# jtschwar/tomo_TV

Hardware: AMD Instinct MI355X
Metric: SART+TV Gvoxel-updates/s (ASD-POCS outer iterations x voxels, 512x512x512 x 90 tilts, at 1/2/4/8 GPU) (higher is better)
Workload: dtype f32; 1 GPU; ASD-POCS iteration (SART sweep beta0=0.25 + 10 TV-GD steps) on ONE 512x512x512 volume, 90 tilts -70..70 deg (headline SART+TV 512^3x90 = BASELINE configs[2] shape), 512 slices on rank 0; volume=512x512x512, slices_per_gpu=512, nray=512, nproj=90, sub_slab_engines_per_gpu=1, sart_chains_per_engine=1

## Files before the change

tomo_tv_amd/csrc/engine_options.inc:

```

int tomo_get_option(tomo_engine *e, const char *name, int *value)
{
    if (!e || !name || !value) return fail(TOMO_ERR_ARG, "null argument");
    if (std::strcmp(name, "fp_strip") == 0) { *value = e->fp_strip; return TOMO_OK; }
    if (std::strcmp(name, "fp_strip_ready") == 0) { *value = e->fs_ok ? 1 : 0; return TOMO_OK; }
    if (std::strcmp(name, "fp_strip_slots") == 0) { *value = e->fs_ok ? e->fs_kused : 0; return TOMO_OK; }
    if (std::strcmp(name, "fp_tile") == 0) { *value = e->fp_tile; return TOMO_OK; }
    if (std::strcmp(name, "bp_tile") == 0) { *value = e->bp_tile; return TOMO_OK; }
    if (std::strcmp(name, "bp_list") == 0) { *value = e->bp_list; return TOMO_OK; }
    if (std::strcmp(name, "fgp_pair") == 0) { *value = e->fgp_pair; return TOMO_OK; }
    if (std::strcmp(name, "fp_list") == 0) { *value = e->fp_list; return TOMO_OK; }
    if (std::strcmp(name, "fp_list_ready") == 0) { *value = e->fl_ok ? 1 : 0; return TOMO_OK; }
    if (std::strcmp(name, "bp_list_ready") == 0) { *value = e->bl_ok ? 1 : 0; return TOMO_OK; }
    if (std::strcmp(name, "fp_reuse") == 0) { *value = e->fp_reuse; return TOMO_OK; }
    if (std::strcmp(name, "art_chain_ready") == 0) { *value = e->art_chain_ok ? 1 : 0; return TOMO_OK; }
    if (std::strcmp(name, "sart_tile") == 0) { *value = e->sart_tile; return TOMO_OK; }
    if (std::strcmp(name, "sart_resident") == 0) { *value = e->sart_resident; return TOMO_OK; }
    if (std::strcmp(name, "sart_resident_ready") == 0) { *value = e->rs_ok ? 1 : 0; return TOMO_OK; }
    if (std::strcmp(name, "sart_resident_active") == 0) { *value = (e->rs_ok && e->sart_resident != 0) ? 1 : 0; return TOMO_OK; }
    if (std::strcmp(name, "sart_resident_spin") == 0) { *value = (int)std::min<uint32_t>(e->rs_spin_limit, 0x7FFFFFFFu); return TOMO_OK; }
    if (std::strcmp(name, "sart_resident_fallbacks") == 0) { *value = e->rs_fallbacks; return TOMO_OK; }
    if (std::strcmp(name, "sart_resident_fallback_chunks") == 0) { *value = e->rs_fallback_chunks; return TOMO_OK; }
    if (std::strcmp(name, "sart_resident_skip") == 0) { *value = e->rs_skip; return TOMO_OK; }
    if (std::strcmp(name, "sart_resident_last_code") == 0) { *value = e->rs_last_code; return TOMO_OK; }
    if (std::strcmp(name, "table_kib") == 0) { *value = (int)std::min<size_t>(e->table_bytes >> 10, 0x7FFFFFFF); return TOMO_OK; }
    if (std::strcmp(name, "create_ms") == 0) { *value = (int)std::min(e->create_ms + 0.5, 2147483647.0); return TOMO_OK; }
    if (std::strcmp(name, "tv_halo_fold") == 0) { *value = e->tv_halo_fold; return TOMO_OK; }
    if (std::strcmp(name, "form_fp") == 0) { *value = select_forms(e).fp; return TOMO_OK; }
    if (std::strcmp(name, "form_bp") == 0) { *value = select_forms(e).bp; return TOMO_OK; }
    if (std::strcmp(name, "form_sart") == 0) { *value = select_forms(e).sart; return TOMO_OK; }
    if (std::strcmp(name, "rccl_version") == 0) { *value = g_rccl.version; return TOMO_OK; }
    if (std::strcmp(name, "comm_rounds") == 0) { *value = (int)std::min<int64_t>(e->comm_rounds, 0x7FFFFFFF); return TOMO_OK; }
    return fail(TOMO_ERR_ARG, std::string("unknown option ") + name);
}

int tomo_set_option(tomo_engine *e, const char *name, int value)
{
    if (!e || !name) return fail(TOMO_ERR_ARG, "null argument");
    if (std::strcmp(name, "fgp_fused") == 0) { e->fgp_fused = value ? 1 : 0; return TOMO_OK; }
    if (std::strcmp(name, "fgp_pair") == 0) { e->fgp_pair = value ? 1 : 0; return TOMO_OK; }
    if (std::strcmp(name, "sart_fused") == 0) { e->sart_fused = value ? 1 : 0; return TOMO_OK; }
    if (std::strcmp(name, "fp_all_lpr") == 0) { e->fp_all_lpr = (value == 16 || value == 32) ? value : 0; return TOMO_OK; }
// ... 19 lines not shown
    if (std::strcmp(name, "fp_tile_chunks_per_pass") == 0) {
        if (value < 0 || e->ft_part || e->ft_part_aux || e->fs_part || e->fs_part_aux || e->fl_part || e->fl_part_aux) return fail(TOMO_ERR_STATE, "fp_tile_chunks_per_pass must be set before the first projection");
        e->ft_ncp_forced = value; e->ft_ncp = 0; e->fs_ncp = 0; e->fl_ncp = 0; return TOMO_OK;
    }
    if (std::strcmp(name, "fp_tile_scratch_mib") == 0) {
        if (value <= 0 || e->ft_part || e->ft_part_aux || e->fs_part || e->fs_part_aux || e->fl_part || e->fl_part_aux) return fail(TOMO_ERR_STATE, "fp_tile_scratch_mib must be positive and set before the first projection");
        e->ft_scratch_cap = (size_t)value << 20; e->ft_ncp = 0; e->fs_ncp = 0; e->fl_ncp = 0; return TOMO_OK;
    }
    if (std::strcmp(name, "tv_gnorm_slot") == 0) {
        if (value < 0 || value >= TOMO_S_COUNT) return fail(TOMO_ERR_ARG, "bad scalar slot");
        e->gnorm_slot = value; return TOMO_OK;
    }
    if (std::strcmp(name, "tv_tz") == 0) { e->tv_tz = value == 4 ? 4 : 8; return TOMO_OK; }
    if (std::strcmp(name, "tv_halo_fold") == 0) { e->tv_halo_fold = value < 0 ? -1 : (value ? 1 : 0); return TOMO_OK; }
    if (std::strcmp(name, "tv_march4") == 0) { e->tv_march4 = value ? 1 : 0; return TOMO_OK; }
    if (std::strcmp(name, "tv_yseg") == 0) { e->tv_yseg = value < 0 ? 0 : value; return TOMO_OK; }
    if (std::strcmp(name, "tv_recompute") == 0) { e->tv_recompute = value ? 1 : 0; return TOMO_OK; }
    if (std::strcmp(name, "tv_lds") == 0) { e->tv_lds = value; return TOMO_OK; }
    return fail(TOMO_ERR_ARG, std::string("unknown option ") + name);
}

int tomo_profile_enable(tomo_engine *e, int kernel, int on)
{
    NEED(e);
    if (kernel < 0 || kernel >= PROF_MAX_KERNELS) return fail(TOMO_ERR_ARG, "bad kernel id");
    HIPCHK(hipStreamSynchronize(e->stream));
    e->prof[kernel].on = on != 0;
    e->prof[kernel].stride = on > 1 ? (unsigned)on : 1u;
    e->prof[kernel].seen = 0;
    e->prof[kernel].used = 0;
// ... 74 lines not shown
```

tomo_tv_amd/csrc/engine_tv.inc:

```

static int field_ptr(tomo_engine *e, int field, float **out)
{
    if (field == TOMO_FIELD_FGP_D) return get_scratch(e, &e->tvg, out);
    if (field == TOMO_FIELD_FGP_P1) return get_scratch(e, &e->fgp_p[0], out);
    return get_vol_ro(e, field, out);
}

int tomo_bind_halo(tomo_engine *e, void *device_lo, void *device_hi)
{
    NEED(e);
    HIPCHK(hipStreamSynchronize(e->stream));
    e->halo_lo = device_lo ? (float *)device_lo : e->halo_lo_own;
    e->halo_hi = device_hi ? (float *)device_hi : e->halo_hi_own;
    return TOMO_OK;
}

int tomo_halo_pack(tomo_engine *e, int field, int last, void *device_dst)
{
    NEED(e);
    float *x; int rc; if ((rc = field_ptr(e, field, &x))) return rc;
    if (!device_dst) return fail(TOMO_ERR_ARG, "null destination");
    hipLaunchKernelGGL(k_halo_pack, dim3((unsigned)((e->npix + 255) / 256)), dim3(256), 0, e->stream, x, (float *)device_dst, (int)e->npix, e->sx, last ? e->nx - 1 : 0);
    LAUNCHCHK();
    return TOMO_OK;
// ... 93 lines not shown
        hipLaunchKernelGGL((k_tv_grad_lds<8, true, false>), grid, dim3(256), 0, e->stream, x, h, (float *)nullptr, (double *)nullptr, eps, e->n, e->nx, e->sx, yseg, e->d_part_tv);
    }
    LAUNCHCHK();
    return part_end(e, e->d_part_tv, TOMO_S_TV);
}

static int tv_rows_per_wave(const tomo_engine *e, int tz)
{
    if (e->tv_yseg > 0) return e->tv_yseg;
    const int64_t cols = (int64_t)((e->n + tz - 1) / tz) * (e->sxc / 64);
    int yseg = 32;
    while (yseg > TV_YSEG_MIN && cols * ((e->n + yseg - 1) / yseg) < TV_WAVES_WANTED) yseg >>= 1;
    return yseg;
}

static int tv_grad_impl(tomo_engine *e, float eps, bool with_tv, float *g_first = nullptr, float *g_last = nullptr)
{
    NEED(e);
    float *x, *g; int rc;
    if ((rc = get_vol(e, e->tv_target, &x))) return rc;
    if ((rc = get_scratch(e, &e->tvg, &g))) return rc;
    if ((rc = reduce_begin(e))) return rc;
    Halo h{e->halo_lo, e->halo_hi};
    if ((g_first || g_last) && !(e->tv_lds == 1 && e->tv_recompute)) return fail(TOMO_ERR_STATE, "gradient planes need the recompute form of the TV march (tv_lds = 1, tv_recompute = 1)");
    if (with_tv && e->tv_lds != 8 && e->tv_lds != 1) with_tv = false;
    if (with_tv) {
        if (!e->d_part_tv) { if ((rc = dev_alloc(e, ENGINE, (void **)&e->d_part_tv, NPART * sizeof(double), true))) return rc; }
        if ((rc = part_begin(e, e->d_part_tv))) return rc;
    }
    {
        ProfScope ps(e, TOMO_K_TV_GRAD);
        e->tv_last_eps = eps;
        double *part_tv = with_tv ? e->d_part_tv : nullptr;
        if (e->tv_lds == 1 && e->tv_recompute) {
            TvUpd gp{};
            gp.wrap_lo = g_last; gp.wrap_hi = g_first;
            const int tz = e->tv_tz == 4 ? 4 : 8, yseg = tv_rows_per_wave(e, tz);
            dim3 grid(tv_march_grid(e->n, tz, e->sxc / 64, (e->n + yseg - 1) / yseg));
            const bool edge = e->nx % 64 != 0 || e->n % 8 != 0;
            with_flag(with_tv, [&](auto W) {
                if (tz == 8 && e->tv_march4) with_flag(edge, [&](auto E) {
                    hipLaunchKernelGGL((k_tv_march4<8, W(), TVM_NORM, E()>), grid, dim3(256), 0, e->stream, x, h, e->d_part, eps, e->n, e->nx, e->sx, yseg, part_tv, gp);
                });
                else with_int<4, 8>(tz, [&](auto TZ) {
                    hipLaunchKernelGGL((k_tv_grad_reg<TZ(), W(), true, TVM_NORM>), grid, dim3(256), 0, e->stream, x, h, (float *)nullptr, e->d_part, eps, e->n, e->nx, e->sx, yseg, part_tv, gp);
                });
            });
        } else if (e->tv_lds == 1) {
            int yseg = 32;
            dim3 grid(tv_march_grid(e->n, 8, e->sxc / 64, (e->n + yseg - 1) / yseg));
            with_flag(with_tv, [&](auto W) {
                hipLaunchKernelGGL((k_tv_grad_reg<8, W()>), grid, dim3(256), 0, e->stream, x, h, g, e->d_part, eps, e->n, e->nx, e->sx, yseg, part_tv, TvUpd{});
            });
        } else if (e->tv_lds) {
            int yseg = 32;
            if (e->tv_lds == 16) {
                dim3 grid((unsigned)(((e->n + 15) / 16) * (e->sxc / 64)), (unsigned)((e->n + yseg - 1) / yseg));
                hipLaunchKernelGGL((k_tv_grad_lds<16, false>), grid, dim3(256), 0, e->stream, x, h, g, e->d_part, eps, e->n, e->nx, e->sx, yseg, (double *)nullptr);
            } else {
                dim3 grid((unsigned)(((e->n + 7) / 8) * (e->sxc / 64)), (unsigned)((e->n + yseg - 1) / yseg));
                with_flag(with_tv, [&](auto W) {
                    hipLaunchKernelGGL((k_tv_grad_lds<8, W()>), grid, dim3(256), 0, e->stream, x, h, g, e->d_part, eps, e->n, e->nx, e->sx, yseg, part_tv);
                });
            }
        } else {
            hipLaunchKernelGGL(k_tv_grad, dim3(tv_grid(e)), dim3(256), 0, e->stream, x, h, g, e->d_part, eps, e->n, e->nx, e->sx);
        }
    }
    LAUNCHCHK();
    if (with_tv && (rc = part_end(e, e->d_part_tv, TOMO_S_TV))) return rc;
    return reduce_end(e, TOMO_S_GNORM);
}

int tomo_tv_set_target(tomo_engine *e, int vol)
{
    NEED(e);
    float *x;
    int rc = get_vol(e, vol, &x);
    if (rc) return rc;
    e->tv_target = vol;
    return TOMO_OK;
}

int tomo_tv_grad(tomo_engine *e, float eps) { return tv_grad_impl(e, eps, false); }
int tomo_tv_grad_tv(tomo_engine *e, float eps)
{
// ... 21 lines not shown
}

static int halo_other_pair(tomo_engine *e, float **lo, float **hi)
{
    int rc;
    if (!e->halo_lo_alt) {
        if ((rc = dev_alloc(e, ENGINE, (void **)&e->halo_lo_alt, e->npix * sizeof(float), true))) return rc;
        if ((rc = dev_alloc(e, ENGINE, (void **)&e->halo_hi_alt, e->npix * sizeof(float), true))) return rc;
    }
    *lo = e->halo_lo == e->halo_lo_own ? e->halo_lo_alt : e->halo_lo_own;
    *hi = e->halo_hi == e->halo_hi_own ? e->halo_hi_alt : e->halo_hi_own;
    return TOMO_OK;
}

static int tv_update_impl(tomo_engine *e, float dPOCS, int clamp, int track_vol, int slot, bool wrap = false,
                          float *plane_last = nullptr, float *plane_first = nullptr, const float *hg_lo = nullptr, const float *hg_hi = nullptr)
{
    NEED(e);
    float *x, *g, *track = nullptr; int rc;
    if ((rc = get_vol(e, e->tv_target, &x))) return rc;
    if ((rc = get_scratch(e, &e->tvg, &g))) return rc;
    if (track_vol >= 0) {
        if (track_vol == e->tv_target) return fail(TOMO_ERR_ARG, "the tracked volume must differ from the one descended");
        if (slot < 0 || slot >= TOMO_S_COUNT) return fail(TOMO_ERR_ARG, "bad scalar slot");
        if ((rc = get_vol(e, track_vol, &track))) return rc;
        if ((rc = order_after_async(e))) return rc;
        if ((rc = reduce_begin(e))) return rc;
    }
    if (e->tv_lds == 1 && e->tv_recompute) {
        float *alt;
        if ((rc = get_scratch(e, &e->tv_alt, &alt))) return rc;
        const bool own_halo = e->halo_lo == e->halo_lo_own || e->halo_lo == e->halo_lo_alt;
        float *wl = plane_last, *wh = plane_first;
        if (wrap && own_halo && (rc = halo_other_pair(e, &wl, &wh))) return rc;
        Halo h{e->halo_lo, e->halo_hi};
        TvUpd up{alt, gnorm_ptr(e), dPOCS, clamp, track, wl, wh, slab_streams(e) ? 1 : 0, nullptr, nullptr, nullptr, nullptr};
        const bool fold = hg_lo && hg_hi && (e->tv_halo_fold < 0 ? e->sxc >= 128 : e->tv_halo_fold != 0) && own_halo && !wrap && e->tv_tz != 4 && e->tv_march4;
        if (fold) {
            up.hg_lo = hg_lo; up.hg_hi = hg_hi;
            if ((rc = halo_other_pair(e, &up.ho_lo, &up.ho_hi))) return rc;
        }
        {
            ProfScope ps(e, TOMO_K_TV_UPDATE);
            const int tz = e->tv_tz == 4 ? 4 : 8, yseg = tv_rows_per_wave(e, tz);
            dim3 grid(tv_march_grid(e->n, tz, e->sxc / 64, (e->n + yseg - 1) / yseg));
            const bool edge = e->nx % 64 != 0 || e->n % 8 != 0;
            if (tz == 8 && e->tv_march4) with_flag(edge, [&](auto E) { with_flag(track != nullptr, [&](auto T) { with_flag(up.stream != 0, [&](auto S) {
                hipLaunchKernelGGL((k_tv_march4<8, false, TVM_UPDATE, E(), T(), S()>), grid, dim3(256), 0, e->stream, x, h, e->d_part, e->tv_last_eps, e->n, e->nx, e->sx, yseg, (double *)nullptr, up);
            }); }); });
            else with_int<4, 8>(tz, [&](auto TZ) {
                hipLaunchKernelGGL((k_tv_grad_reg<TZ(), false, true, TVM_UPDATE>), grid, dim3(256), 0, e->stream, x, h, (float *)nullptr, e->d_part, e->tv_last_eps, e->n, e->nx, e->sx, yseg, (double *)nullptr, up);
            });
        }
        LAUNCHCHK();
        e->vol[e->tv_target] = alt; e->tv_alt = x;
        if (wrap && own_halo) { e->halo_lo = wl; e->halo_hi = wh; }
        else if (wrap) { if ((rc = tomo_halo_local(e, e->tv_target))) return rc; }
        if (fold) { e->halo_lo = up.ho_lo; e->halo_hi = up.ho_hi; }
        else if (hg_lo && hg_hi && (rc = tomo_tv_halo_apply(e, dPOCS, clamp, hg_lo, hg_hi))) return rc;
        return track ? reduce_end(e, slot) : TOMO_OK;
    }
    int64_t n4 = e->vol_elems() / 4;
// ... 76 lines not shown
    return TOMO_OK;
}

int tomo_tv(tomo_engine *e, int vol, float eps)
{
    int rc;
    if ((rc = tomo_halo_local(e, vol))) return rc;
    return tomo_tv_partial(e, vol, eps);
}

static int tv_gd_impl(tomo_engine *e, int ng, float dPOCS, float eps, int track_vol, int slot)
{
    int rc;
    if (!e) return fail(TOMO_ERR_ARG, "null engine");
    const bool fold_tv = ng > 0 && (e->tv_lds == 8 || e->tv_lds == 1);
    if (fold_tv) { if ((rc = tomo_halo_local(e, e->tv_target))) return rc; }
    else if ((rc = tomo_tv(e, e->tv_target, eps))) return rc;
    for (int g = 0; g < ng; ++g) {
        if ((rc = tv_grad_impl(e, eps, fold_tv && g == 0))) return rc;
        if ((rc = tv_update_impl(e, dPOCS, g == ng - 1, g == ng - 1 ? track_vol : -1, slot, g < ng - 1))) return rc;
    }
    if (ng <= 0) {
        if ((rc = tomo_positivity(e, e->tv_target))) return rc;
        if (track_vol >= 0) {
            if ((rc = tomo_diff_norm_sq(e, e->tv_target, track_vol, slot))) return rc;
            return tomo_copy_volume(e, track_vol, e->tv_target);
        }
    }
    return TOMO_OK;
}

int tomo_tv_gd(tomo_engine *e, int ng, float dPOCS, float eps) { return tv_gd_impl(e, ng, dPOCS, eps, -1, 0); }

int tomo_tv_gd_tracked(tomo_engine *e, int ng, float dPOCS, float eps, int track_vol, int slot)
{
// ... 155 lines not shown
```

tomo_tv_amd/csrc/kernels_common.hip.h:

```cpp
#pragma once

namespace tomo {


template <int V> struct VecOf;
template <> struct VecOf<1> { typedef float T; };
template <> struct VecOf<2> { typedef float T __attribute__((ext_vector_type(2))); };
template <> struct VecOf<4> { typedef float T __attribute__((ext_vector_type(4))); };

template <int V> __device__ __forceinline__ typename VecOf<V>::T vzero();
template <> __device__ __forceinline__ float vzero<1>() { return 0.f; }
template <> __device__ __forceinline__ VecOf<2>::T vzero<2>() { VecOf<2>::T v = {0.f, 0.f}; return v; }
template <> __device__ __forceinline__ VecOf<4>::T vzero<4>() { VecOf<4>::T v = {0.f, 0.f, 0.f, 0.f}; return v; }

template <int V> __device__ __forceinline__ float velem(const typename VecOf<V>::T &v, int i);
template <> __device__ __forceinline__ float velem<1>(const float &v, int) { return v; }
template <> __device__ __forceinline__ float velem<2>(const VecOf<2>::T &v, int i) { return v[i]; }
template <> __device__ __forceinline__ float velem<4>(const VecOf<4>::T &v, int i) { return v[i]; }

template <int V> __device__ __forceinline__ void vset(typename VecOf<V>::T &v, int i, float f);
template <> __device__ __forceinline__ void vset<1>(float &v, int, float f) { v = f; }
template <> __device__ __forceinline__ void vset<2>(VecOf<2>::T &v, int i, float f) { v[i] = f; }
template <> __device__ __forceinline__ void vset<4>(VecOf<4>::T &v, int i, float f) { v[i] = f; }

// ... 40 lines not shown
__global__ void k_finalize(double *__restrict__ part, double *__restrict__ dst)
{
    double v = part[threadIdx.x];
    part[threadIdx.x] = 0.0;
    __shared__ double red[NPART / 64];
    v = wave_sum(v);
    if ((threadIdx.x & 63) == 0) red[threadIdx.x >> 6] = v;
    __syncthreads();
    if (threadIdx.x == 0) {
        double s = 0;
        for (int i = 0; i < NPART / 64; ++i) s += red[i];
        *dst = s;
    }
}

__global__ __launch_bounds__(256) void k_transpose_in(const float *__restrict__ src, float *__restrict__ dst,
                                                       int ns, int64_t m, int sx)
{
    __shared__ float tile[32][33];
    int64_t m0 = (int64_t)blockIdx.x * 32;
    int s0 = blockIdx.y * 32;
    int tx = threadIdx.x & 31, ty = threadIdx.x >> 5;
    for (int r = ty; r < 32; r += 8) {
        int s = s0 + r;
        int64_t mm = m0 + tx;
        tile[r][tx] = (s < ns && mm < m) ? src[(int64_t)s * m + mm] : 0.f;
    }
    __syncthreads();
    for (int r = ty; r < 32; r += 8) {
        int64_t mm = m0 + r;
// ... 43 lines not shown
```

tomo_tv_amd/csrc/kernels_tv.hip.h:

```cpp
#pragma once

namespace tomo {

struct Halo { const float *lo; const float *hi; };

__device__ __forceinline__ float ldx(const float *__restrict__ x, const Halo &h, int pix, int s, int nx, int sx)
{
    if (s < 0) return h.lo[pix];
    if (s >= nx) return h.hi[pix];
    return x[(size_t)pix * sx + s];
}

__global__ void k_halo_pack(const float *__restrict__ x, float *__restrict__ dst, int npix, int sx, int s)
{
    int i = blockIdx.x * blockDim.x + threadIdx.x;
    if (i < npix) dst[i] = x[(size_t)i * sx + s];
}

__global__ void k_scalars_to_host(const double *__restrict__ src, double *__restrict__ host_dst, int n)
{
    int i = threadIdx.x;
    if (i < n) host_dst[i] = src[i];
}

// ... 172 lines not shown
}

__device__ __forceinline__ float tv_step_len(float dPOCS, const double *gnorm2) { return fminf(__fdiv_rn(dPOCS, (float)sqrt(*gnorm2)), 3.402823466e38f); }
__device__ __forceinline__ float tv_step(float c, float gv, float len) { return __fmaf_rn(-gv, len, c); }

constexpr int TVL_TZ = 8;
constexpr int TVL_PITCH = 66;

__device__ __forceinline__ float tv_ld(const float *__restrict__ x, const Halo &h, int pix, int s, int nx, int sx)
{
    const float *p = x + (size_t)pix * sx + s;
    p = (s < 0) ? h.lo + pix : p;
    p = (s >= nx) ? h.hi + pix : p;
    return *p;
}

template <int TZ, bool WITH_TV, bool GRAD = true>
__global__ __launch_bounds__(256) void k_tv_grad_lds(const float *__restrict__ x, Halo h, float *__restrict__ g,
                                                      double *__restrict__ part, float eps, int n, int nx, int sx,
                                                      int yseg, double *__restrict__ part_tv)
{
    __shared__ float ring[4][TZ + 2][TVL_PITCH];
    __shared__ float rinv[2][TZ + 1][TVL_PITCH];
    const int lane = threadIdx.x & 63, wave = threadIdx.x >> 6;
    const int nzb = (n + TZ - 1) / TZ;
    int bz = blockIdx.x % nzb;
    int bs = blockIdx.x / nzb;
    int y0 = blockIdx.y * yseg;
    int y1 = min(y0 + yseg, n);
    int z0 = bz * TZ, s0 = bs * 64;
// ... 75 lines not shown
        __syncthreads();
        block_accumulate(tvacc, part_tv);
    }
}

inline unsigned tv_march_grid(int n, int tz, int nchunk, int nys)
{
    const int nzb = (n + tz - 1) / tz;
    if ((nzb & 7) == 0) return 8u * (unsigned)(((int64_t)(nzb >> 3) * nchunk * nys + 3) / 4);
    return (unsigned)(((int64_t)nzb * nchunk * nys + 3) / 4);
}

enum { TVM_STORE = 0, TVM_NORM = 1, TVM_UPDATE = 2, TVM_VALUE = 3 };
struct TvUpd { float *x_out; const double *gnorm2; float dPOCS; int clamp; float *track; float *wrap_lo; float *wrap_hi;
               int stream;
               const float *hg_lo; const float *hg_hi; float *ho_lo; float *ho_hi; };

template <int TZ, bool WITH_TV, bool GRAD = true, int MODE = TVM_STORE>
__global__ __launch_bounds__(256) void k_tv_grad_reg(const float *__restrict__ x, Halo h, float *__restrict__ g,
                                                      double *__restrict__ part, float eps, int n, int nx, int sx,
                                                      int yseg, double *__restrict__ part_tv, TvUpd up = TvUpd{})
{
    const int lane = threadIdx.x & 63, wave = __builtin_amdgcn_readfirstlane(threadIdx.x >> 6);
    const int nzb = (n + TZ - 1) / TZ, nchunk = (nx + 63) >> 6   , nys = (n + yseg - 1) / yseg;
    double acc = 0.0, tvacc = 0.0;
    float nrm_ = 1.f;
    if (MODE == TVM_UPDATE) nrm_ = tv_step_len(up.dPOCS, up.gnorm2);
    int bs, bz, ys;
    bool live;
    if ((nzb & 7) == 0) {
        const int zpx = nzb >> 3;
// ... 134 lines not shown
        __syncthreads();
        block_accumulate(tvacc, part_tv);
    }
}

#ifndef TV4_PACKED
#define TV4_PACKED 1
#endif
#ifndef TV4_PACKED_EDGE
#define TV4_PACKED_EDGE 0
#endif
#ifndef TV4_UPD_WAVES
#define TV4_UPD_WAVES 4
#endif
#define TV4_OCC __attribute__((amdgpu_waves_per_eu((MODE == TVM_UPDATE && !TRACK) ? TV4_UPD_WAVES : 4, (MODE == TVM_UPDATE && !TRACK) ? TV4_UPD_WAVES : 8)))
template <int TZ, bool WITH_TV, int MODE, bool EDGE, bool TRACK = false, bool STREAM = false>
__global__ __launch_bounds__(256) TV4_OCC void k_tv_march4(const float *__restrict__ x, Halo h, double *__restrict__ part, float eps,
                                                    int n, int nx, int sx, int yseg, double *__restrict__ part_tv, TvUpd up)
{
    static_assert(MODE == TVM_NORM || MODE == TVM_UPDATE || MODE == TVM_VALUE, "modes without a stored gradient");
    static_assert(MODE != TVM_VALUE || WITH_TV, "the value mode sums the TV integrand");
    const int lane = threadIdx.x & 63, wave = __builtin_amdgcn_readfirstlane(threadIdx.x >> 6);
    const int nzb = (n + TZ - 1) / TZ, nchunk = (nx + 63) >> 6   , nys = (n + yseg - 1) / yseg;
    double acc = 0.0, tvacc = 0.0;
    float nrm_ = 1.f;
    if (MODE == TVM_UPDATE) nrm_ = tv_step_len(up.dPOCS, up.gnorm2);
    int bs, bz, ys;
    if ((nzb & 7) == 0) {
        const int zpx = nzb >> 3;
        const int64_t li = (int64_t)(blockIdx.x >> 3) * 4 + wave;
        bs = (int)(li % nchunk); bz = (int)(blockIdx.x & 7) * zpx + (int)((li / nchunk) % zpx); ys = (int)(li / ((int64_t)nchunk * zpx));
    } else {
        const int64_t item = (int64_t)blockIdx.x * 4 + wave;
        bs = (int)(item % nchunk); bz = (int)((item / nchunk) % nzb); ys = (int)(item / ((int64_t)nchunk * nzb));
    }
    if (ys < nys) {
        const int y0 = ys * yseg, y1 = min(y0 + yseg, n);
        const int z0 = bz * TZ, s0 = bs * 64, s = s0 + lane;
        int zc[TZ + 2];
#pragma unroll
        for (int j = 0; j < TZ + 2; ++j) { int z = (z0 - 1 + j) % n; zc[j] = z < 0 ? z + n : z; }
        int zl;
        { int z = (z0 - 1 + (lane < TZ + 2 ? lane : 0)) % n; zl = z < 0 ? z + n : z; }
        auto yrow = [&](int y) { int r = y % n; return r < 0 ? r + n : r; };
        float rows[4][TZ + 2], Ta[TZ + 1], Tb[TZ + 1];
        float pe[4], pf[4], pc[4];
        const bool lo_in = s0 > 0, hi_in = s0 + 64 < nx;
        const unsigned zls = (unsigned)zl * (unsigned)sx;
        const unsigned off_lo = lo_in ? zls + (unsigned)(s0 - 1) : (unsigned)zl, off_hi = hi_in ? zls + (unsigned)(s0 + 64) : (unsigned)zl;
        constexpr bool SOFF = !EDGE && !(WITH_TV && MODE == TVM_NORM);
        unsigned vb[TZ + 2];
#pragma unroll
        for (int j = 0; j < TZ + 2; ++j) vb[j] = ((unsigned)zc[j] * (unsigned)sx + (unsigned)s0 + (unsigned)lane) * 4u;
        unsigned eb_c = (zls + (unsigned)s0) * 4u, eb_lo = off_lo * 4u, eb_hi = off_hi * 4u;
        auto fetch = [&](int y, float *c, float &e_lo, float &e_hi, float &e_c) __attribute__((always_inline)) {
            int yy = yrow(y) * n;
            if (!EDGE) {
                const float *rowp = x + (size_t)yy * sx;
                if constexpr (SOFF) {
                    const SBase rb = sgpr_base(rowp);
#pragma unroll
                    for (int j = 0; j < TZ + 2; ++j) c[j] = ld_so(rb, vb[j]);
                    e_c = ld_so(rb, eb_c);
                    e_lo = ld_so(sgpr_base(lo_in ? rowp : h.lo + yy), eb_lo);
                    e_hi = ld_so(sgpr_base(hi_in ? rowp : h.hi + yy), eb_hi);
                } else {
#pragma unroll
                    for (int j = 0; j < TZ + 2; ++j) c[j] = (rowp + ((unsigned)zc[j] * (unsigned)sx + (unsigned)s0))[(unsigned)lane];
                    e_c = rowp[zls + (unsigned)s0];
                    e_lo = (lo_in ? rowp : h.lo + yy)[off_lo];
                    e_hi = (hi_in ? rowp : h.hi + yy)[off_hi];
                }
            } else {
#pragma unroll
                for (int j = 0; j < TZ + 2; ++j) c[j] = tv_ld(x, h, yy + zc[j], s, nx, sx);
                e_lo = tv_ld(x, h, yy + zl, s0 - 1, nx, sx);
                e_hi = tv_ld(x, h, yy + zl, s0 + 64, nx, sx);
                e_c = tv_ld(x, h, yy + zl, s0, nx, sx);
            }
        };
        const float vmin = up.clamp ? 0.f : -INFINITY;
        const bool planes = up.wrap_lo != nullptr && (EDGE || s0 == 0 || s0 + 64 == nx);
#define TV4_RINV(C, IP, JP, KP, RR, DD, D1, D2, D3)                                                       \
        {                                                                                                 \
            D1 = (C) - (IP); D2 = (C) - (JP); D3 = (C) - (KP);                                            \
            float q_ = __fmaf_rn(D3, D3, __fmaf_rn(D2, D2, __fmaf_rn(D1, D1, eps)));                      \
            RR = tv_rsqrt(q_);                                                                            \
// ... 132 lines not shown
                        else if (STREAM) __builtin_nontemporal_store(out[j], tr_e + (size_t)(j - 1) * sx + (unsigned)lane);
                        else (tr_e + (size_t)(j - 1) * sx)[(unsigned)lane] = out[j];
                    }
                }
            }
            if (planes) {
                if (s == 0) {
#pragma unroll
                    for (int j = 1; j <= TZ; ++j) if (!EDGE || z0 + j - 1 < n) up.wrap_hi[pix0 + (j - 1)] = out[j];
                }
                if (s == nx - 1) {
#pragma unroll
                    for (int j = 1; j <= TZ; ++j) if (!EDGE || z0 + j - 1 < n) up.wrap_lo[pix0 + (j - 1)] = out[j];
                }
            }
            if (MODE == TVM_UPDATE && up.hg_lo != nullptr && (EDGE || s0 == 0 || s0 + 64 == nx)) {
                if (!EDGE) {
                    const unsigned hp = (unsigned)(y * n) + (unsigned)zl;
                    if (lane >= 1 && lane <= TZ) {
                        if (s0 == 0) up.ho_lo[hp] = fmaxf(tv_step(pe0, up.hg_lo[hp], nrm_), vmin);
                        if (s0 + 64 == nx) up.ho_hi[hp] = fmaxf(tv_step(pf0, up.hg_hi[hp], nrm_), vmin);
                    }
                } else {
                    if (s == 0) {
#pragma unroll
                        for (int j = 1; j <= TZ; ++j)
                            if (z0 + j - 1 < n) up.ho_lo[pix0 + (j - 1)] = fmaxf(tv_step(h.lo[pix0 + (j - 1)], up.hg_lo[pix0 + (j - 1)], nrm_), vmin);
                    }
                    if (s == nx - 1) {
#pragma unroll
// ... 78 lines not shown
```

tomo_tv_amd/csrc/tomo_engine.hip:

```cpp
#include "../../include/tomo_hip.h"
#include "kernels.hip.h"
#include "sart_resident.hip.h"
#include "sysmat.h"
#include "resident.h"
#include "dev_pool.h"

#include <dlfcn.h>
#if __has_include(<rccl/rccl.h>)
#include <rccl/rccl.h>
#else
#define NCCL_UNIQUE_ID_BYTES 128
typedef struct ncclComm *ncclComm_t;
typedef struct { char internal[NCCL_UNIQUE_ID_BYTES]; } ncclUniqueId;
typedef enum { ncclSuccess = 0 } ncclResult_t;
typedef enum { ncclFloat32 = 7, ncclFloat64 = 8 } ncclDataType_t;
typedef enum { ncclSum = 0 } ncclRedOp_t;
#endif

#include <algorithm>
#include <atomic>
#include <chrono>
#include <cmath>
#include <condition_variable>
#include <functional>
// ... 89 lines not shown
    uint32_t *d_rptr = nullptr;
    uint2 *d_rent = nullptr;
    float *d_rowsum = nullptr, *d_rowinner = nullptr, *d_colsum_all = nullptr, *d_rowcross = nullptr;
    bool art_chain_ok = false;
    int art_chain = 1;
    CellD *d_cell = nullptr;
    uint32_t *d_wptr = nullptr;
    uint2 *d_went = nullptr;
    float lipschitz = 0.f, lipschitz_cimmino = 0.f;
    int sart_fused = 1;
    int tv_lds = 1, fp_all_lpr = 16;
    int tv_recompute = 1, tv_tz = 8;
    int tv_yseg = 0;
    int tv_march4 = 1;
    int tv_halo_fold = -1;
    int gnorm_slot = TOMO_S_GNORM;
    double *gnorm_override = nullptr;
    hipEvent_t ev_peer = nullptr;
    float tv_last_eps = 1e-6f;
    float *tv_alt = nullptr, *halo_lo_alt = nullptr, *halo_hi_alt = nullptr;
    SegItemD *d_seg_exec = nullptr;
    std::vector<uint32_t> h_seg_exec_ptr;
    uint32_t *d_row_first = nullptr, *d_row_nseg = nullptr;
    float *seg_partial = nullptr;
    uint32_t max_items = 0;
    bool seg_ready = false;
    std::vector<double> angles;
    float *sart_alt = nullptr;
    int fp_tile = 1, ft_tiles_z = 0, ft_ntiles = 0;
    uint32_t ft_nseg = 0;
// ... 86 lines not shown
    float *cg_coef = nullptr;
    float *tvg = nullptr;
    float *fgp_p[3] = {nullptr, nullptr, nullptr};
    float *fgp_q[3] = {nullptr, nullptr, nullptr};
    int fgp_fused = 1;
    int fgp_pair = 1;
    float *pdhg_p[3] = {nullptr, nullptr, nullptr}, *pdhg_alt[4] = {nullptr, nullptr, nullptr, nullptr}, *pdhg_q = nullptr;
    bool pdhg_begun = false;
    float *stage = nullptr;
    size_t stage_bytes = 0;
    double *d_scal = nullptr, *d_scal_own = nullptr, *d_part = nullptr, *d_part_aux = nullptr, *d_part_tv = nullptr;
    double *h_snap = nullptr;
    hipEvent_t ev_snap = nullptr;
    bool snap_pending = false;
    bool part_open[3] = {false, false, false};
    hipStream_t aux = nullptr;
    hipEvent_t ev_fork = nullptr, ev_join = nullptr;
    bool async_pending = false;
    struct CommRef *comm = nullptr;
    int64_t comm_rounds = 0;
    float *comm_send_first = nullptr, *comm_send_last = nullptr, *comm_g_lo = nullptr, *comm_g_hi = nullptr;
    float *comm_fgp = nullptr;
    double *comm_scal = nullptr;
    uint64_t vol_version[TOMO_VOL_SLOTS] = {};
    struct { int vol = -1; uint64_t ver = 0; } g_valid[2];
    int fp_reuse = 1;
    float *g_prev = nullptr;
    float *g_yk = nullptr;
    struct { bool valid = false; uint64_t ver = 0; } yk_claim;
    bool g_prev_valid = false, mom_p_ok = false;
// ... 134 lines not shown
}
static int part_begin(tomo_engine *e, double *part)
{
    bool &open = part_open(e, part);
    if (open) HIPCHK(hipMemsetAsync(part, 0, NPART * sizeof(double), e->stream));
    open = true;
    return TOMO_OK;
}
static int part_end(tomo_engine *e, double *part, int slot)
{
    hipLaunchKernelGGL(k_finalize, dim3(1), dim3(NPART), 0, e->stream, part, e->d_scal + slot);
    LAUNCHCHK();
    part_open(e, part) = false;
    return TOMO_OK;
}
static int reduce_begin(tomo_engine *e) { return part_begin(e, e->d_part); }
static int reduce_end(tomo_engine *e, int slot) { return part_end(e, e->d_part, slot); }

constexpr int TV_YSEG_MIN = 8, TV_WAVES_WANTED = 4096;
static int grid_1d(int64_t n4) { int64_t b = (n4 + 255) / 256; return (int)std::min<int64_t>(std::max<int64_t>(b, 1), 4096); }

#include "engine_launch.inc"
#include "engine_create.inc"

extern "C" {

#include "engine_api.inc"
#include "engine_tv.inc"
#include "engine_pdhg.inc"
#include "engine_comm.inc"
// ... 4 lines not shown
```

Measured before the change: 10.61 Gvoxel-updates/s.

## Fold TV gradient-norm finalize into update kernel and self-wrap first halo

In the plain single-GPU TV descent, the gradient-norm partial sums now go to double-buffered partial arrays. Each update kernel block reduces them itself, which removes the separate finalize launch and memset between norm and update passes. The next buffer is zeroed inside the norm kernel. The first norm pass can also read periodic x-neighbours directly from the volume and write the halo planes itself, skipping the separate halo_local step. The cost is a redundant per-block reduction of NPART doubles in every update block, plus extra template instantiations.

```diff
diff --git a/tomo_tv_amd/csrc/engine_options.inc b/tomo_tv_amd/csrc/engine_options.inc
--- a/tomo_tv_amd/csrc/engine_options.inc
+++ b/tomo_tv_amd/csrc/engine_options.inc
@@ -26,6 +26,19 @@
     if (std::strcmp(name, "table_kib") == 0) { *value = (int)std::min<size_t>(e->table_bytes >> 10, 0x7FFFFFFF); return TOMO_OK; }
     if (std::strcmp(name, "create_ms") == 0) { *value = (int)std::min(e->create_ms + 0.5, 2147483647.0); return TOMO_OK; }
     if (std::strcmp(name, "tv_halo_fold") == 0) { *value = e->tv_halo_fold; return TOMO_OK; }
+    if (std::strcmp(name, "tv_fold_sums") == 0) { *value = e->tv_fold_sums; return TOMO_OK; }
+    if (std::strcmp(name, "tv_self_wrap") == 0) { *value = e->tv_self_wrap; return TOMO_OK; }
+    if (std::strcmp(name, "tv_fold_sums_dirty") == 0) {
+        *value = -1;
+        if (!e->d_part_gn[0] || !e->d_part_gn[1]) return TOMO_OK;
+        double h[2 * NPART];
+        HIPCHK(hipSetDevice(e->device));
+        HIPCHK(hipStreamSynchronize(e->stream));
+        for (int k = 0; k < 2; ++k) HIPCHK(hipMemcpy(h + k * NPART, e->d_part_gn[k], NPART * sizeof(double), hipMemcpyDeviceToHost));
+        *value = 0;
+        for (double v : h) if (!(v == 0.0)) ++*value;
+        return TOMO_OK;
+    }
     if (std::strcmp(name, "form_fp") == 0) { *value = select_forms(e).fp; return TOMO_OK; }
     if (std::strcmp(name, "form_bp") == 0) { *value = select_forms(e).bp; return TOMO_OK; }
     if (std::strcmp(name, "form_sart") == 0) { *value = select_forms(e).sart; return TOMO_OK; }
@@ -75,6 +88,8 @@
     if (std::strcmp(name, "tv_tz") == 0) { e->tv_tz = value == 4 ? 4 : 8; return TOMO_OK; }
     if (std::strcmp(name, "tv_halo_fold") == 0) { e->tv_halo_fold = value < 0 ? -1 : (value ? 1 : 0); return TOMO_OK; }
     if (std::strcmp(name, "tv_march4") == 0) { e->tv_march4 = value ? 1 : 0; return TOMO_OK; }
+    if (std::strcmp(name, "tv_fold_sums") == 0) { e->tv_fold_sums = value < 0 ? -1 : (value ? 1 : 0); return TOMO_OK; }
+    if (std::strcmp(name, "tv_self_wrap") == 0) { e->tv_self_wrap = value < 0 ? -1 : (value ? 1 : 0); return TOMO_OK; }
     if (std::strcmp(name, "tv_yseg") == 0) { e->tv_yseg = value < 0 ? 0 : value; return TOMO_OK; }
     if (std::strcmp(name, "tv_recompute") == 0) { e->tv_recompute = value ? 1 : 0; return TOMO_OK; }
     if (std::strcmp(name, "tv_lds") == 0) { e->tv_lds = value; return TOMO_OK; }
diff --git a/tomo_tv_amd/csrc/engine_tv.inc b/tomo_tv_amd/csrc/engine_tv.inc
--- a/tomo_tv_amd/csrc/engine_tv.inc
+++ b/tomo_tv_amd/csrc/engine_tv.inc
@@ -131,13 +131,23 @@
     return yseg;
 }
 
-static int tv_grad_impl(tomo_engine *e, float eps, bool with_tv, float *g_first = nullptr, float *g_last = nullptr)
+static bool tv_plain_descent(const tomo_engine *e)
+{
+    const bool own_lo = e->halo_lo == e->halo_lo_own || (e->halo_lo_alt && e->halo_lo == e->halo_lo_alt);
+    const bool own_hi = e->halo_hi == e->halo_hi_own || (e->halo_hi_alt && e->halo_hi == e->halo_hi_alt);
+    return e->tv_lds == 1 && e->tv_recompute && e->tv_march4 && e->tv_tz != 4 && own_lo && own_hi &&
+           !e->gnorm_override && !e->comm && e->gnorm_slot == TOMO_S_GNORM;
+}
+
+static int tv_grad_impl(tomo_engine *e, float eps, bool with_tv, float *g_first = nullptr, float *g_last = nullptr,
+                        double *gn_part = nullptr, double *gn_zero = nullptr, bool self_wrap = false)
 {
     NEED(e);
     float *x, *g; int rc;
+    if ((gn_part || gn_zero || self_wrap) && (!tv_plain_descent(e) || g_first || g_last || (self_wrap && !with_tv))) return fail(TOMO_ERR_STATE, "not the whole-volume form of the TV descent");
     if ((rc = get_vol(e, e->tv_target, &x))) return rc;
     if ((rc = get_scratch(e, &e->tvg, &g))) return rc;
-    if ((rc = reduce_begin(e))) return rc;
+    if (!gn_part && (rc = reduce_begin(e))) return rc;
     Halo h{e->halo_lo, e->halo_hi};
     if ((g_first || g_last) && !(e->tv_lds == 1 && e->tv_recompute)) return fail(TOMO_ERR_STATE, "gradient planes need the recompute form of the TV march (tv_lds = 1, tv_recompute = 1)");
     if (with_tv && e->tv_lds != 8 && e->tv_lds != 1) with_tv = false;
@@ -152,12 +162,18 @@
         if (e->tv_lds == 1 && e->tv_recompute) {
             TvUpd gp{};
             gp.wrap_lo = g_last; gp.wrap_hi = g_first;
+            gp.zero_part = gn_zero;
+            if (self_wrap) { gp.ho_lo = e->halo_lo; gp.ho_hi = e->halo_hi; }
+            double *part = gn_part ? gn_part : e->d_part;
             const int tz = e->tv_tz == 4 ? 4 : 8, yseg = tv_rows_per_wave(e, tz);
             dim3 grid(tv_march_grid(e->n, tz, e->sxc / 64, (e->n + yseg - 1) / yseg));
             const bool edge = e->nx % 64 != 0 || e->n % 8 != 0;
-            with_flag(with_tv, [&](auto W) {
+            if (self_wrap) with_flag(edge, [&](auto E) {
+                hipLaunchKernelGGL((k_tv_march4<8, true, TVM_NORM, E(), false, false, true>), grid, dim3(256), 0, e->stream, x, h, part, eps, e->n, e->nx, e->sx, yseg, part_tv, gp);
+            });
+            else with_flag(with_tv, [&](auto W) {
                 if (tz == 8 && e->tv_march4) with_flag(edge, [&](auto E) {
-                    hipLaunchKernelGGL((k_tv_march4<8, W(), TVM_NORM, E()>), grid, dim3(256), 0, e->stream, x, h, e->d_part, eps, e->n, e->nx, e->sx, yseg, part_tv, gp);
+                    hipLaunchKernelGGL((k_tv_march4<8, W(), TVM_NORM, E()>), grid, dim3(256), 0, e->stream, x, h, part, eps, e->n, e->nx, e->sx, yseg, part_tv, gp);
                 });
                 else with_int<4, 8>(tz, [&](auto TZ) {
                     hipLaunchKernelGGL((k_tv_grad_reg<TZ(), W(), true, TVM_NORM>), grid, dim3(256), 0, e->stream, x, h, (float *)nullptr, e->d_part, eps, e->n, e->nx, e->sx, yseg, part_tv, gp);
@@ -186,7 +202,7 @@
     }
     LAUNCHCHK();
     if (with_tv && (rc = part_end(e, e->d_part_tv, TOMO_S_TV))) return rc;
-    return reduce_end(e, TOMO_S_GNORM);
+    return gn_part ? TOMO_OK : reduce_end(e, TOMO_S_GNORM);
 }
 
 int tomo_tv_set_target(tomo_engine *e, int vol)
@@ -238,10 +254,12 @@
 }
 
 static int tv_update_impl(tomo_engine *e, float dPOCS, int clamp, int track_vol, int slot, bool wrap = false,
-                          float *plane_last = nullptr, float *plane_first = nullptr, const float *hg_lo = nullptr, const float *hg_hi = nullptr)
+                          float *plane_last = nullptr, float *plane_first = nullptr, const float *hg_lo = nullptr, const float *hg_hi = nullptr,
+                          const double *gn_part = nullptr)
 {
     NEED(e);
     float *x, *g, *track = nullptr; int rc;
+    if (gn_part && (!tv_plain_descent(e) || track_vol >= 0 || hg_lo || hg_hi)) return fail(TOMO_ERR_STATE, "not the whole-volume form of the TV descent");
     if ((rc = get_vol(e, e->tv_target, &x))) return rc;
     if ((rc = get_scratch(e, &e->tvg, &g))) return rc;
     if (track_vol >= 0) {
@@ -259,6 +277,7 @@
         if (wrap && own_halo && (rc = halo_other_pair(e, &wl, &wh))) return rc;
         Halo h{e->halo_lo, e->halo_hi};
         TvUpd up{alt, gnorm_ptr(e), dPOCS, clamp, track, wl, wh, slab_streams(e) ? 1 : 0, nullptr, nullptr, nullptr, nullptr};
+        if (gn_part) { up.gnorm2 = gn_part; up.gnorm_out = e->d_scal + e->gnorm_slot; }
         const bool fold = hg_lo && hg_hi && (e->tv_halo_fold < 0 ? e->sxc >= 128 : e->tv_halo_fold != 0) && own_halo && !wrap && e->tv_tz != 4 && e->tv_march4;
         if (fold) {
             up.hg_lo = hg_lo; up.hg_hi = hg_hi;
@@ -269,7 +288,10 @@
             const int tz = e->tv_tz == 4 ? 4 : 8, yseg = tv_rows_per_wave(e, tz);
             dim3 grid(tv_march_grid(e->n, tz, e->sxc / 64, (e->n + yseg - 1) / yseg));
             const bool edge = e->nx % 64 != 0 || e->n % 8 != 0;
-            if (tz == 8 && e->tv_march4) with_flag(edge, [&](auto E) { with_flag(track != nullptr, [&](auto T) { with_flag(up.stream != 0, [&](auto S) {
+            if (gn_part) with_flag(edge, [&](auto E) { with_flag(up.stream != 0, [&](auto S) {
+                hipLaunchKernelGGL((k_tv_march4<8, false, TVM_UPDATE, E(), false, S(), false, true>), grid, dim3(256), 0, e->stream, x, h, e->d_part, e->tv_last_eps, e->n, e->nx, e->sx, yseg, (double *)nullptr, up);
+            }); });
+            else if (tz == 8 && e->tv_march4) with_flag(edge, [&](auto E) { with_flag(track != nullptr, [&](auto T) { with_flag(up.stream != 0, [&](auto S) {
                 hipLaunchKernelGGL((k_tv_march4<8, false, TVM_UPDATE, E(), T(), S()>), grid, dim3(256), 0, e->stream, x, h, e->d_part, e->tv_last_eps, e->n, e->nx, e->sx, yseg, (double *)nullptr, up);
             }); }); });
             else with_int<4, 8>(tz, [&](auto TZ) {
@@ -376,11 +398,16 @@
     int rc;
     if (!e) return fail(TOMO_ERR_ARG, "null engine");
     const bool fold_tv = ng > 0 && (e->tv_lds == 8 || e->tv_lds == 1);
-    if (fold_tv) { if ((rc = tomo_halo_local(e, e->tv_target))) return rc; }
+    const bool plain = ng > 0 && tv_plain_descent(e);
+    const bool self_wrap = plain && fold_tv && e->tv_self_wrap != 0, fold_sums = plain && ng > 1 && e->tv_fold_sums != 0;
+    if (fold_tv) { if (!self_wrap && (rc = tomo_halo_local(e, e->tv_target))) return rc; }
     else if ((rc = tomo_tv(e, e->tv_target, eps))) return rc;
+    if (fold_sums && (rc = gn_begin(e))) return rc;
     for (int g = 0; g < ng; ++g) {
-        if ((rc = tv_grad_impl(e, eps, fold_tv && g == 0))) return rc;
-        if ((rc = tv_update_impl(e, dPOCS, g == ng - 1, g == ng - 1 ? track_vol : -1, slot, g < ng - 1))) return rc;
+        double *gn_part = fold_sums && g < ng - 1 ? e->d_part_gn[g & 1] : nullptr, *gn_zero = fold_sums ? e->d_part_gn[(g + 1) & 1] : nullptr;
+        if ((rc = tv_grad_impl(e, eps, fold_tv && g == 0, nullptr, nullptr, gn_part, gn_zero, self_wrap && g == 0))) return rc;
+        if (fold_sums && g == ng - 1) gn_end(e);
+        if ((rc = tv_update_impl(e, dPOCS, g == ng - 1, g == ng - 1 ? track_vol : -1, slot, g < ng - 1, nullptr, nullptr, nullptr, nullptr, gn_part))) return rc;
     }
     if (ng <= 0) {
         if ((rc = tomo_positivity(e, e->tv_target))) return rc;
diff --git a/tomo_tv_amd/csrc/kernels_common.hip.h b/tomo_tv_amd/csrc/kernels_common.hip.h
--- a/tomo_tv_amd/csrc/kernels_common.hip.h
+++ b/tomo_tv_amd/csrc/kernels_common.hip.h
@@ -78,6 +78,17 @@
     }
 }
 
+__device__ __forceinline__ double block_sum_parts(const double *part)
+{
+    __shared__ double red[NPART / 64];
+    double v = wave_sum(part[threadIdx.x]);
+    if ((threadIdx.x & 63) == 0) red[threadIdx.x >> 6] = v;
+    __syncthreads();
+    double s = 0;
+    for (int i = 0; i < NPART / 64; ++i) s += red[i];
+    return s;
+}
+
 __global__ __launch_bounds__(256) void k_transpose_in(const float *__restrict__ src, float *__restrict__ dst,
                                                        int ns, int64_t m, int sx)
 {
diff --git a/tomo_tv_amd/csrc/kernels_tv.hip.h b/tomo_tv_amd/csrc/kernels_tv.hip.h
--- a/tomo_tv_amd/csrc/kernels_tv.hip.h
+++ b/tomo_tv_amd/csrc/kernels_tv.hip.h
@@ -210,6 +210,10 @@
     p = (s >= nx) ? h.hi + pix : p;
     return *p;
 }
+__device__ __forceinline__ float tv_ld_wrap(const float *__restrict__ x, int pix, int s, int nx, int sx)
+{
+    return x[(size_t)pix * sx + (s < 0 ? nx - 1 : (s >= nx ? 0 : s))];
+}
 
 template <int TZ, bool WITH_TV, bool GRAD = true>
 __global__ __launch_bounds__(256) void k_tv_grad_lds(const float *__restrict__ x, Halo h, float *__restrict__ g,
@@ -315,7 +319,8 @@
 enum { TVM_STORE = 0, TVM_NORM = 1, TVM_UPDATE = 2, TVM_VALUE = 3 };
 struct TvUpd { float *x_out; const double *gnorm2; float dPOCS; int clamp; float *track; float *wrap_lo; float *wrap_hi;
                int stream;
-               const float *hg_lo; const float *hg_hi; float *ho_lo; float *ho_hi; };
+               const float *hg_lo; const float *hg_hi; float *ho_lo; float *ho_hi;
+               double *gnorm_out; double *zero_part; };
 
 template <int TZ, bool WITH_TV, bool GRAD = true, int MODE = TVM_STORE>
 __global__ __launch_bounds__(256) void k_tv_grad_reg(const float *__restrict__ x, Halo h, float *__restrict__ g,
@@ -480,17 +485,26 @@
 #define TV4_UPD_WAVES 4
 #endif
 #define TV4_OCC __attribute__((amdgpu_waves_per_eu((MODE == TVM_UPDATE && !TRACK) ? TV4_UPD_WAVES : 4, (MODE == TVM_UPDATE && !TRACK) ? TV4_UPD_WAVES : 8)))
-template <int TZ, bool WITH_TV, int MODE, bool EDGE, bool TRACK = false, bool STREAM = false>
+template <int TZ, bool WITH_TV, int MODE, bool EDGE, bool TRACK = false, bool STREAM = false, bool SELFWRAP = false, bool FOLD = false>
 __global__ __launch_bounds__(256) TV4_OCC void k_tv_march4(const float *__restrict__ x, Halo h, double *__restrict__ part, float eps,
                                                     int n, int nx, int sx, int yseg, double *__restrict__ part_tv, TvUpd up)
 {
     static_assert(MODE == TVM_NORM || MODE == TVM_UPDATE || MODE == TVM_VALUE, "modes without a stored gradient");
     static_assert(MODE != TVM_VALUE || WITH_TV, "the value mode sums the TV integrand");
+    static_assert(!SELFWRAP || MODE != TVM_UPDATE, "the update pass reads the planes the norm pass used");
+    static_assert(!FOLD || (MODE == TVM_UPDATE && !TRACK), "the partial sums are added up by an untracked update pass");
     const int lane = threadIdx.x & 63, wave = __builtin_amdgcn_readfirstlane(threadIdx.x >> 6);
     const int nzb = (n + TZ - 1) / TZ, nchunk = (nx + 63) >> 6   , nys = (n + yseg - 1) / yseg;
     double acc = 0.0, tvacc = 0.0;
     float nrm_ = 1.f;
-    if (MODE == TVM_UPDATE) nrm_ = tv_step_len(up.dPOCS, up.gnorm2);
+    if (MODE == TVM_UPDATE) {
+        if constexpr (FOLD) {
+            const double g2 = block_sum_parts(up.gnorm2);
+            if (blockIdx.x == 0 && threadIdx.x == 0) *up.gnorm_out = g2;
+            nrm_ = tv_step_len(up.dPOCS, &g2);
+        } else nrm_ = tv_step_len(up.dPOCS, up.gnorm2);
+    }
+    if (MODE == TVM_NORM && up.zero_part != nullptr && blockIdx.x == 0) up.zero_part[threadIdx.x] = 0.0;
     int bs, bz, ys;
     if ((nzb & 7) == 0) {
         const int zpx = nzb >> 3;
@@ -513,7 +527,8 @@
         float pe[4], pf[4], pc[4];
         const bool lo_in = s0 > 0, hi_in = s0 + 64 < nx;
         const unsigned zls = (unsigned)zl * (unsigned)sx;
-        const unsigned off_lo = lo_in ? zls + (unsigned)(s0 - 1) : (unsigned)zl, off_hi = hi_in ? zls + (unsigned)(s0 + 64) : (unsigned)zl;
+        const unsigned off_lo = lo_in ? zls + (unsigned)(s0 - 1) : (SELFWRAP ? zls + (unsigned)(nx - 1) : (unsigned)zl);
+        const unsigned off_hi = hi_in ? zls + (unsigned)(s0 + 64) : (SELFWRAP ? zls : (unsigned)zl);
         constexpr bool SOFF = !EDGE && !(WITH_TV && MODE == TVM_NORM);
         unsigned vb[TZ + 2];
 #pragma unroll
@@ -528,15 +543,21 @@
 #pragma unroll
                     for (int j = 0; j < TZ + 2; ++j) c[j] = ld_so(rb, vb[j]);
                     e_c = ld_so(rb, eb_c);
-                    e_lo = ld_so(sgpr_base(lo_in ? rowp : h.lo + yy), eb_lo);
-                    e_hi = ld_so(sgpr_base(hi_in ? rowp : h.hi + yy), eb_hi);
+                    e_lo = ld_so(sgpr_base((SELFWRAP || lo_in) ? rowp : h.lo + yy), eb_lo);
+                    e_hi = ld_so(sgpr_base((SELFWRAP || hi_in) ? rowp : h.hi + yy), eb_hi);
                 } else {
 #pragma unroll
                     for (int j = 0; j < TZ + 2; ++j) c[j] = (rowp + ((unsigned)zc[j] * (unsigned)sx + (unsigned)s0))[(unsigned)lane];
                     e_c = rowp[zls + (unsigned)s0];
-                    e_lo = (lo_in ? rowp : h.lo + yy)[off_lo];
-                    e_hi = (hi_in ? rowp : h.hi + yy)[off_hi];
-                }
+                    e_lo = ((SELFWRAP || lo_in) ? rowp : h.lo + yy)[off_lo];
+                    e_hi = ((SELFWRAP || hi_in) ? rowp : h.hi + yy)[off_hi];
+                }
+            } else if constexpr (SELFWRAP) {
+#pragma unroll
+                for (int j = 0; j < TZ + 2; ++j) c[j] = tv_ld_wrap(x, yy + zc[j], s, nx, sx);
+                e_lo = tv_ld_wrap(x, yy + zl, s0 - 1, nx, sx);
+                e_hi = tv_ld_wrap(x, yy + zl, s0 + 64, nx, sx);
+                e_c = tv_ld_wrap(x, yy + zl, s0, nx, sx);
             } else {
 #pragma unroll
                 for (int j = 0; j < TZ + 2; ++j) c[j] = tv_ld(x, h, yy + zc[j], s, nx, sx);
@@ -699,6 +720,16 @@
                     for (int j = 1; j <= TZ; ++j) if (!EDGE || z0 + j - 1 < n) up.wrap_lo[pix0 + (j - 1)] = out[j];
                 }
             }
+            if (SELFWRAP && MODE == TVM_NORM && (EDGE || s0 == 0 || s0 + 64 == nx)) {
+                if (s == 0) {
+#pragma unroll
+                    for (int j = 1; j <= TZ; ++j) if (!EDGE || z0 + j - 1 < n) up.ho_hi[pix0 + (j - 1)] = c0[j];
+                }
+                if (s == nx - 1) {
+#pragma unroll
+                    for (int j = 1; j <= TZ; ++j) if (!EDGE || z0 + j - 1 < n) up.ho_lo[pix0 + (j - 1)] = c0[j];
+                }
+            }
             if (MODE == TVM_UPDATE && up.hg_lo != nullptr && (EDGE || s0 == 0 || s0 + 64 == nx)) {
                 if (!EDGE) {
                     const unsigned hp = (unsigned)(y * n) + (unsigned)zl;
diff --git a/tomo_tv_amd/csrc/tomo_engine.hip b/tomo_tv_amd/csrc/tomo_engine.hip
--- a/tomo_tv_amd/csrc/tomo_engine.hip
+++ b/tomo_tv_amd/csrc/tomo_engine.hip
@@ -127,6 +127,7 @@
     int tv_yseg = 0;
     int tv_march4 = 1;
     int tv_halo_fold = -1;
+    int tv_fold_sums = -1, tv_self_wrap = -1;
     int gnorm_slot = TOMO_S_GNORM;
     double *gnorm_override = nullptr;
     hipEvent_t ev_peer = nullptr;
@@ -243,6 +244,8 @@
     hipEvent_t ev_snap = nullptr;
     bool snap_pending = false;
     bool part_open[3] = {false, false, false};
+    double *d_part_gn[2] = {nullptr, nullptr};
+    bool gn_open = false;
     hipStream_t aux = nullptr;
     hipEvent_t ev_fork = nullptr, ev_join = nullptr;
     bool async_pending = false;
@@ -407,6 +410,16 @@
     part_open(e, part) = false;
     return TOMO_OK;
 }
+static int gn_begin(tomo_engine *e)
+{
+    for (int k = 0; k < 2; ++k) {
+        if (!e->d_part_gn[k]) { if (int rc = dev_alloc(e, ENGINE, (void **)&e->d_part_gn[k], NPART * sizeof(double), true)) return rc; }
+        else if (e->gn_open) HIPCHK(hipMemsetAsync(e->d_part_gn[k], 0, NPART * sizeof(double), e->stream));
+    }
+    e->gn_open = true;
+    return TOMO_OK;
+}
+static void gn_end(tomo_engine *e) { e->gn_open = false; }
 static int reduce_begin(tomo_engine *e) { return part_begin(e, e->d_part); }
 static int reduce_end(tomo_engine *e, int slot) { return part_end(e, e->d_part, slot); }
 
```

Measured after the change: 10.64 Gvoxel-updates/s, median of 6. Within noise of the previous version (+0.3%).
